# rampasek/GraphGPS

Measured on NVIDIA H100. Metric: graphs/sec GPSLayer fwd+bwd, higher is better.
Workload: dtype f32

## Files before the change

graphgps_b200/csrc/attention.cu:

```cuda
#include "kernels.cuh"

namespace gps {

namespace {

constexpr int kWarpsPerBlock = 4;

__device__ __forceinline__ int find_graph(const int* __restrict__ gptr, int B, int node) {
  int lo = 0, hi = B;
  while (hi - lo > 1) {
    int mid = (lo + hi) >> 1;
    if (gptr[mid] <= node) lo = mid; else hi = mid;
  }
  return lo;
}

template <int LPR>
__device__ __forceinline__ float group_sum(float v) {
#pragma unroll
  for (int o = LPR / 2; o > 0; o >>= 1) v += __shfl_xor_sync(0xffffffffu, v, o);
  return v;
}

__device__ __forceinline__ int warp_max_i(int v) {
#pragma unroll
  for (int o = 16; o > 0; o >>= 1) v = max(v, __shfl_xor_sync(0xffffffffu, v, o));
  return v;
}

struct DropQuad {
  Philox4 r;
  uint32_t thr;
  float keep_scale;
};
__device__ __forceinline__ void drop_quad_refresh(DropQuad& q, float p, uint64_t seed, uint64_t offset, int head, int i, int jl) {
  q.r = philox4x32(seed, offset + (uint64_t)(GPS_SITE_ATTN_P + head), ((uint64_t)i << 20) | (uint64_t)(jl >> 2));
}
__device__ __forceinline__ float drop_quad_scale(const DropQuad& q, int jl) {
  const int k = jl & 3;
  const uint32_t bits = k == 0 ? q.r.v[0] : k == 1 ? q.r.v[1] : k == 2 ? q.r.v[2] : q.r.v[3];
  return bits >= q.thr ? q.keep_scale : 0.f;
}
__device__ __forceinline__ void drop_quad_init(DropQuad& q, float p) {
  q.thr = (uint32_t)fminf(p * 4294967296.f, 4294967295.f);
  q.keep_scale = 1.f / (1.f - p);
}

template <int CH, int LPR>
__device__ __forceinline__ void load_slice(float4* dst, const float* row, int sub, int nch, bool ok) {
#pragma unroll
  for (int c = 0; c < CH; ++c) {
    int ch = sub + c * LPR;
    dst[c] = (ok && ch < nch) ? ld4(row + ch * 4) : f4zero();
  }
}
template <int CH, int LPR>
__device__ __forceinline__ void store_slice(const float4* src, float* row, int sub, int nch) {
#pragma unroll
  for (int c = 0; c < CH; ++c) {
    int ch = sub + c * LPR;
    if (ch < nch) st4(row + ch * 4, src[c]);
  }
}
template <int CH, int LPR>
__device__ __forceinline__ void store_slice_planes(const float4* src, const Planes& p, int64_t r, int64_t col0, int sub, int nch) {
  if (!p.hi) return;
#pragma unroll
  for (int c = 0; c < CH; ++c) {
    int ch = sub + c * LPR;
    if (ch < nch) planes_store4(p, r, col0 + ch * 4, src[c]);
  }
}
template <int CH>
__device__ __forceinline__ float dot_slice(const float4* a, const float4* b) {
  float s = 0.f;
#pragma unroll
  for (int c = 0; c < CH; ++c) s += a[c].x * b[c].x + a[c].y * b[c].y + a[c].z * b[c].z + a[c].w * b[c].w;
  return s;
}

struct AttnArgs {
  const int* gptr; int B; int N; int H; int hd;
  const float* Q; const float* K; const float* V; int64_t ld;
  float* O; const float* Oc; const float* dO; int64_t ldo;
  float* lse; const float* lsec; float* delta; const float* deltac;
  float* dQ; float* dK; float* dV; int64_t ldg;
  float scale; float p_drop; uint64_t seed, offset;
  const unsigned long long* offset_dev;
  Planes Op, dQp, dKp, dVp;
  int smem_rows;
};
__device__ __forceinline__ uint64_t eff_offset(const AttnArgs& a) {
  return a.offset + ((a.p_drop > 0.f && a.offset_dev) ? *a.offset_dev : 0ull);
}

struct StagedRows {
  const float* x; int64_t ldx;
  const float* y; int64_t ldy;
};
template <int RPB>
__device__ __forceinline__ StagedRows stage_rows(const AttnArgs& a, const float* X, int64_t ldX, const float* Y, int64_t ldY,
                                                 int h, float* sm) {
  const int64_t hoff = (int64_t)h * a.hd;
  StagedRows r{X + hoff, ldX, Y + hoff, ldY};
  const int r0 = blockIdx.x * RPB;
  if (a.smem_rows <= 0 || r0 >= a.N) return r;
  const int last = min(r0 + RPB, a.N) - 1;
  const int kmin = a.gptr[find_graph(a.gptr, a.B, r0)];
  const int R = a.gptr[find_graph(a.gptr, a.B, last) + 1] - kmin;
  if (R > a.smem_rows) return r;
  const int pitch = a.hd + 4, nch = a.hd >> 2;
  float* sx = sm;
  float* sy = sm + (int64_t)a.smem_rows * pitch;
  for (int idx = threadIdx.x; idx < R * nch; idx += blockDim.x) {
    const int row = idx / nch, c = idx - row * nch;
    st4(sx + row * pitch + c * 4, ld4(X + (int64_t)(kmin + row) * ldX + hoff + c * 4));
    st4(sy + row * pitch + c * 4, ld4(Y + (int64_t)(kmin + row) * ldY + hoff + c * 4));
  }
  __syncthreads();
  r.x = sx - (int64_t)kmin * pitch; r.ldx = pitch;
  r.y = sy - (int64_t)kmin * pitch; r.ldy = pitch;
  return r;
}

template <int CH, int LPR>
__global__ void __launch_bounds__(kWarpsPerBlock * 32) k_attn_fwd(AttnArgs a) {
  extern __shared__ float attn_sm[];
  constexpr int RPW = 32 / LPR;
  const int warp = threadIdx.x >> 5, lane = threadIdx.x & 31;
  const int sub = lane % LPR, rloc = lane / LPR;
  const int h = blockIdx.y;
  const int i = (blockIdx.x * kWarpsPerBlock + warp) * RPW + rloc;
  const bool row_ok = i < a.N;
  const int nch = a.hd / 4;
  const uint64_t offs = eff_offset(a);
  int gs = 0, n = 0;
  if (row_ok) {
    int g = find_graph(a.gptr, a.B, i);
    gs = a.gptr[g];
    n = a.gptr[g + 1] - gs;
  }
  const int nloop = warp_max_i(n);
  const int64_t hoff = (int64_t)h * a.hd;
  float4 q[CH], o[CH];
  load_slice<CH, LPR>(q, a.Q + (int64_t)(row_ok ? i : 0) * a.ld + hoff, sub, nch, row_ok);
#pragma unroll
  for (int c = 0; c < CH; ++c) {
    q[c] = f4scale(q[c], a.scale);
    o[c] = f4zero();
  }
  float m = -INFINITY, l = 0.f;
  const bool use_drop = a.p_drop > 0.f;
  DropQuad dq;
  drop_quad_init(dq, a.p_drop);
  const StagedRows kv = stage_rows<RPW * kWarpsPerBlock>(a, a.K, a.ld, a.V, a.ld, h, attn_sm);
  float4 kc[CH], vc[CH];
  load_slice<CH, LPR>(kc, kv.x + (int64_t)gs * kv.ldx, sub, nch, n > 0);
  load_slice<CH, LPR>(vc, kv.y + (int64_t)gs * kv.ldy, sub, nch, n > 0);
  for (int jl = 0; jl < nloop; ++jl) {
    if (use_drop && (jl & 3) == 0) drop_quad_refresh(dq, a.p_drop, a.seed, offs, h, i, jl);
    const bool valid = jl < n;
    const bool nvalid = jl + 1 < n;
    const int jn = gs + (nvalid ? jl + 1 : 0);
    float4 kn[CH], vn[CH];
    load_slice<CH, LPR>(kn, kv.x + (int64_t)jn * kv.ldx, sub, nch, nvalid);
    load_slice<CH, LPR>(vn, kv.y + (int64_t)jn * kv.ldy, sub, nch, nvalid);
    float s = group_sum<LPR>(dot_slice<CH>(q, kc));
    s = valid ? s : -INFINITY;
    const float m_new = fmaxf(m, s);
    const float corr = (m_new == -INFINITY) ? 1.f : __expf(m - m_new);
    const float p = valid ? __expf(s - m_new) : 0.f;
    l = l * corr + p;
    const float pd = use_drop ? p * drop_quad_scale(dq, jl) : p;
#pragma unroll
    for (int c = 0; c < CH; ++c) {
      o[c].x = o[c].x * corr + pd * vc[c].x;
      o[c].y = o[c].y * corr + pd * vc[c].y;
      o[c].z = o[c].z * corr + pd * vc[c].z;
      o[c].w = o[c].w * corr + pd * vc[c].w;
      kc[c] = kn[c];
      vc[c] = vn[c];
    }
    m = m_new;
  }
  if (row_ok) {
    const float inv = 1.f / l;
#pragma unroll
    for (int c = 0; c < CH; ++c) o[c] = f4scale(o[c], inv);
    store_slice<CH, LPR>(o, a.O + (int64_t)i * a.ldo + hoff, sub, nch);
    store_slice_planes<CH, LPR>(o, a.Op, i, hoff, sub, nch);
    if (sub == 0) a.lse[(int64_t)i * a.H + h] = m + __logf(l);
  }
}

__global__ void k_attn_delta(AttnArgs a) {
  const int64_t t = ((int64_t)blockIdx.x * blockDim.x + threadIdx.x) >> 3;
  const int sub = threadIdx.x & 7;
  const bool ok = t < (int64_t)a.N * a.H;
  const int64_t i = ok ? t / a.H : 0;
  const int h = ok ? (int)(t - i * a.H) : 0;
  const float4* go = reinterpret_cast<const float4*>(a.dO + i * a.ldo + (int64_t)h * a.hd);
  const float4* oo = reinterpret_cast<const float4*>(a.Oc + i * a.ldo + (int64_t)h * a.hd);
  float acc = 0.f;
  if (ok)
    for (int c = sub; c < a.hd / 4; c += 8) {
      const float4 x = __ldg(go + c), y = __ldg(oo + c);
      acc += x.x * y.x + x.y * y.y + x.z * y.z + x.w * y.w;
    }
  acc += __shfl_xor_sync(0xffffffffu, acc, 4);
  acc += __shfl_xor_sync(0xffffffffu, acc, 2);
  acc += __shfl_xor_sync(0xffffffffu, acc, 1);
  if (ok && sub == 0) a.delta[t] = acc;
}

template <int CH, int LPR>
__device__ __forceinline__ void attn_bwd_q_body(const AttnArgs& a, float* attn_sm) {
  constexpr int RPW = 32 / LPR;
  const int warp = threadIdx.x >> 5, lane = threadIdx.x & 31;
  const int sub = lane % LPR, rloc = lane / LPR;
  const int h = blockIdx.y;
  const int i = (blockIdx.x * kWarpsPerBlock + warp) * RPW + rloc;
  const bool row_ok = i < a.N;
  const int nch = a.hd / 4;
  const uint64_t offs = eff_offset(a);
  int gs = 0, n = 0;
  if (row_ok) {
    int g = find_graph(a.gptr, a.B, i);
    gs = a.gptr[g];
    n = a.gptr[g + 1] - gs;
  }
  const int nloop = warp_max_i(n);
  const int64_t hoff = (int64_t)h * a.hd;
  const int ir = row_ok ? i : 0;
  float4 q[CH], go[CH], gq[CH];
  load_slice<CH, LPR>(q, a.Q + (int64_t)ir * a.ld + hoff, sub, nch, row_ok);
  load_slice<CH, LPR>(go, a.dO + (int64_t)ir * a.ldo + hoff, sub, nch, row_ok);
  {
    const float dl = row_ok ? a.deltac[(int64_t)i * a.H + h] : 0.f;
#pragma unroll
    for (int c = 0; c < CH; ++c) gq[c] = f4zero();
    const float lse = row_ok ? a.lsec[(int64_t)i * a.H + h] : 0.f;
#pragma unroll
    for (int c = 0; c < CH; ++c) q[c] = f4scale(q[c], a.scale);
    const bool use_drop = a.p_drop > 0.f;
    DropQuad dq;
    drop_quad_init(dq, a.p_drop);
    const StagedRows kv = stage_rows<RPW * kWarpsPerBlock>(a, a.K, a.ld, a.V, a.ld, h, attn_sm);
    float4 kk[CH], vv[CH];
    load_slice<CH, LPR>(kk, kv.x + (int64_t)gs * kv.ldx, sub, nch, n > 0);
    load_slice<CH, LPR>(vv, kv.y + (int64_t)gs * kv.ldy, sub, nch, n > 0);
    for (int jl = 0; jl < nloop; ++jl) {
      if (use_drop && (jl & 3) == 0) drop_quad_refresh(dq, a.p_drop, a.seed, offs, h, i, jl);
      const bool valid = jl < n;
      const bool nvalid = jl + 1 < n;
      const int jn = gs + (nvalid ? jl + 1 : 0);
      float4 kn[CH], vn[CH];
      load_slice<CH, LPR>(kn, kv.x + (int64_t)jn * kv.ldx, sub, nch, nvalid);
      load_slice<CH, LPR>(vn, kv.y + (int64_t)jn * kv.ldy, sub, nch, nvalid);
      float s = dot_slice<CH>(q, kk), dp = dot_slice<CH>(go, vv);
#pragma unroll
      for (int ofs = LPR / 2; ofs > 0; ofs >>= 1) {
        s += __shfl_xor_sync(0xffffffffu, s, ofs);
        dp += __shfl_xor_sync(0xffffffffu, dp, ofs);
      }
      const float p = valid ? __expf(s - lse) : 0.f;
      const float ds = p * (dp * (use_drop ? drop_quad_scale(dq, jl) : 1.f) - dl);
#pragma unroll
      for (int c = 0; c < CH; ++c) {
        gq[c].x += ds * kk[c].x;
        gq[c].y += ds * kk[c].y;
        gq[c].z += ds * kk[c].z;
        gq[c].w += ds * kk[c].w;
        kk[c] = kn[c];
        vv[c] = vn[c];
      }
    }
  }
  if (row_ok) {
#pragma unroll
    for (int c = 0; c < CH; ++c) gq[c] = f4scale(gq[c], a.scale);
    store_slice<CH, LPR>(gq, a.dQ + (int64_t)i * a.ldg + hoff, sub, nch);
    store_slice_planes<CH, LPR>(gq, a.dQp, i, hoff, sub, nch);
  }
}

template <int CH, int LPR>
__device__ __forceinline__ void attn_bwd_kv_body(const AttnArgs& a, float* attn_sm) {
  constexpr int RPW = 32 / LPR;
  const int warp = threadIdx.x >> 5, lane = threadIdx.x & 31;
  const int sub = lane % LPR, rloc = lane / LPR;
  const int h = blockIdx.y;
  const int j = (blockIdx.x * kWarpsPerBlock + warp) * RPW + rloc;
  const bool row_ok = j < a.N;
  const int nch = a.hd / 4;
  const uint64_t offs = eff_offset(a);
  int gs = 0, n = 0;
  if (row_ok) {
    int g = find_graph(a.gptr, a.B, j);
    gs = a.gptr[g];
    n = a.gptr[g + 1] - gs;
  }
  const int nloop = warp_max_i(n);
  const int jl = j - gs;
  const int64_t hoff = (int64_t)h * a.hd;
  const int jr = row_ok ? j : 0;
  float4 kk[CH], vv[CH], gk[CH], gv[CH];
  load_slice<CH, LPR>(kk, a.K + (int64_t)jr * a.ld + hoff, sub, nch, row_ok);
  load_slice<CH, LPR>(vv, a.V + (int64_t)jr * a.ld + hoff, sub, nch, row_ok);
#pragma unroll
  for (int c = 0; c < CH; ++c) {
    gk[c] = f4zero();
    gv[c] = f4zero();
  }
  const StagedRows qd = stage_rows<RPW * kWarpsPerBlock>(a, a.Q, a.ld, a.dO, a.ldo, h, attn_sm);
  float4 q[CH], go[CH];
  load_slice<CH, LPR>(q, qd.x + (int64_t)gs * qd.ldx, sub, nch, n > 0);
  load_slice<CH, LPR>(go, qd.y + (int64_t)gs * qd.ldy, sub, nch, n > 0);
  for (int il = 0; il < nloop; ++il) {
    const bool valid = il < n;
    const int i = gs + (valid ? il : 0);
    const bool nvalid = il + 1 < n;
    const int in_ = gs + (nvalid ? il + 1 : 0);
    float4 qn[CH], gon[CH];
    load_slice<CH, LPR>(qn, qd.x + (int64_t)in_ * qd.ldx, sub, nch, nvalid);
    load_slice<CH, LPR>(gon, qd.y + (int64_t)in_ * qd.ldy, sub, nch, nvalid);
    float s = dot_slice<CH>(q, kk), dp = dot_slice<CH>(go, vv);
#pragma unroll
    for (int ofs = LPR / 2; ofs > 0; ofs >>= 1) {
      s += __shfl_xor_sync(0xffffffffu, s, ofs);
      dp += __shfl_xor_sync(0xffffffffu, dp, ofs);
    }
    const float lse = valid ? a.lsec[(int64_t)i * a.H + h] : 0.f;
    const float dl = valid ? a.deltac[(int64_t)i * a.H + h] : 0.f;
    const float p = valid ? __expf(s * a.scale - lse) : 0.f;
    float dsc = 1.f;
    if (a.p_drop > 0.f) {
      DropQuad dq;
      drop_quad_init(dq, a.p_drop);
      drop_quad_refresh(dq, a.p_drop, a.seed, offs, h, i, jl);
      dsc = drop_quad_scale(dq, jl);
    }
    const float pd = p * dsc;
    const float ds = p * (dp * dsc - dl) * a.scale;
#pragma unroll
    for (int c = 0; c < CH; ++c) {
      gk[c].x += ds * q[c].x; gk[c].y += ds * q[c].y; gk[c].z += ds * q[c].z; gk[c].w += ds * q[c].w;
      gv[c].x += pd * go[c].x; gv[c].y += pd * go[c].y; gv[c].z += pd * go[c].z; gv[c].w += pd * go[c].w;
      q[c] = qn[c];
      go[c] = gon[c];
    }
  }
  if (row_ok) {
    store_slice<CH, LPR>(gk, a.dK + (int64_t)j * a.ldg + hoff, sub, nch);
    store_slice<CH, LPR>(gv, a.dV + (int64_t)j * a.ldg + hoff, sub, nch);
    store_slice_planes<CH, LPR>(gk, a.dKp, j, hoff, sub, nch);
    store_slice_planes<CH, LPR>(gv, a.dVp, j, hoff, sub, nch);
  }
}

template <int CH, int LPR>
__global__ void __launch_bounds__(kWarpsPerBlock * 32) k_attn_bwd(AttnArgs a) {
  extern __shared__ float attn_sm[];
  if (blockIdx.z == 0) attn_bwd_kv_body<CH, LPR>(a, attn_sm);
  else attn_bwd_q_body<CH, LPR>(a, attn_sm);
}

enum { KFWD = 0, KBWD = 1 };

constexpr int kStageBytes = 72 * 1024;

template <int CH, int LPR>
static void launch_one(int which, const AttnArgs& a0, cudaStream_t stream) {
  constexpr int RPW = 32 / LPR;
  AttnArgs a = a0;
  static const bool stage_on = [] {
    const char* e = getenv("GPS_B200_ATTN_STAGE");
    return e && e[0] == '1';
  }();
  const int pitch = a.hd + 4;
  a.smem_rows = (stage_on && a.B > 0 && a.N < 64LL * a.B) ? kStageBytes / (2 * pitch * 4) : 0;
  const size_t smem = a.smem_rows > 0 ? (size_t)2 * a.smem_rows * pitch * 4 : 0;
  static bool attr_done[2] = {false, false};
  if (smem > 0 && !attr_done[which]) {
    if (which == KFWD) cudaFuncSetAttribute(k_attn_fwd<CH, LPR>, cudaFuncAttributeMaxDynamicSharedMemorySize, kStageBytes);
    else cudaFuncSetAttribute(k_attn_bwd<CH, LPR>, cudaFuncAttributeMaxDynamicSharedMemorySize, kStageBytes);
    attr_done[which] = true;
  }
  dim3 grid((unsigned)ceil_div(a.N, (int64_t)RPW * kWarpsPerBlock), (unsigned)a.H, which == KFWD ? 1 : 2);
  dim3 block(kWarpsPerBlock * 32);
  if (which == KFWD) k_attn_fwd<CH, LPR><<<grid, block, smem, stream>>>(a);
  else k_attn_bwd<CH, LPR><<<grid, block, smem, stream>>>(a);
}

static int dispatch(int which, const AttnArgs& a, cudaStream_t stream) {
  GPS_REQUIRE(a.hd > 0 && a.hd % 4 == 0, GPS_ERR_UNSUPPORTED, "attention: head dim %d must be a multiple of 4", a.hd);
  GPS_REQUIRE(a.ld % 4 == 0 && a.ldo % 4 == 0 && (which == KFWD || a.ldg % 4 == 0), GPS_ERR_UNSUPPORTED,
              "attention: leading dimensions must be multiples of 4");
  const int nch = a.hd / 4;
  GPS_REQUIRE(nch <= 48, GPS_ERR_UNSUPPORTED, "attention: head dim %d > 192 not supported", a.hd);
  if (a.N == 0) return GPS_OK;
  int lpr = 1;
  while ((nch + lpr - 1) / lpr > 6) lpr *= 2;
  const int ch = (nch + lpr - 1) / lpr;
#define GPS_ATTN_CASE(CHV, LPRV)                                  \
  if (ch == CHV && lpr == LPRV) {                                 \
    launch_one<CHV, LPRV>(which, a, stream);                      \
    GPS_LAUNCH_CHECK();                                           \
    return GPS_OK;                                                \
  }
  GPS_ATTN_CASE(1, 1) GPS_ATTN_CASE(2, 1) GPS_ATTN_CASE(3, 1) GPS_ATTN_CASE(4, 1) GPS_ATTN_CASE(5, 1)
  GPS_ATTN_CASE(6, 1) GPS_ATTN_CASE(4, 2) GPS_ATTN_CASE(5, 2) GPS_ATTN_CASE(6, 2) GPS_ATTN_CASE(4, 4)
  GPS_ATTN_CASE(5, 4) GPS_ATTN_CASE(6, 4) GPS_ATTN_CASE(4, 8) GPS_ATTN_CASE(5, 8) GPS_ATTN_CASE(6, 8)
#undef GPS_ATTN_CASE
  set_error("attention: no kernel for head dim %d", a.hd);
  return GPS_ERR_UNSUPPORTED;
}

}

int attention_fwd(const GpsGraph& g, int64_t heads, int64_t hd, const float* Q, const float* K, const float* V,
                  int64_t ld, float* O, int64_t ldo, float* lse, float p_drop, uint64_t seed, uint64_t offset,
                  cudaStream_t stream, const unsigned long long* offset_dev, Planes Op) {
  AttnArgs a{};
  a.offset_dev = offset_dev;
  a.Op = Op;
  a.gptr = g.graph_ptr; a.B = (int)g.B; a.N = (int)g.N; a.H = (int)heads; a.hd = (int)hd;
  a.Q = Q; a.K = K; a.V = V; a.ld = ld; a.O = O; a.ldo = ldo; a.lse = lse;
  a.scale = 1.f / sqrtf((float)hd); a.p_drop = p_drop; a.seed = seed; a.offset = offset;
  return dispatch(KFWD, a, stream);
}

int attention_bwd(const GpsGraph& g, int64_t heads, int64_t hd, const float* Q, const float* K, const float* V,
                  int64_t ld, const float* O, const float* dO, int64_t ldo, const float* lse, float* delta,
                  float* dQ, float* dK, float* dV, int64_t ldg, float p_drop, uint64_t seed, uint64_t offset,
                  cudaStream_t stream, const unsigned long long* offset_dev, Planes dQp, Planes dKp, Planes dVp) {
  AttnArgs a{};
  a.offset_dev = offset_dev;
  a.dQp = dQp; a.dKp = dKp; a.dVp = dVp;
  a.gptr = g.graph_ptr; a.B = (int)g.B; a.N = (int)g.N; a.H = (int)heads; a.hd = (int)hd;
  a.Q = Q; a.K = K; a.V = V; a.ld = ld; a.Oc = O; a.dO = dO; a.ldo = ldo; a.lsec = lse;
  a.delta = delta; a.deltac = delta; a.dQ = dQ; a.dK = dK; a.dV = dV; a.ldg = ldg;
  a.scale = 1.f / sqrtf((float)hd); a.p_drop = p_drop; a.seed = seed; a.offset = offset;
  if (a.N == 0) return GPS_OK;
  const int64_t nt = (int64_t)a.N * a.H * 8;
  k_attn_delta<<<(unsigned)ceil_div(nt, (int64_t)256), 256, 0, stream>>>(a);
  GPS_LAUNCH_CHECK();
  return dispatch(KBWD, a, stream);
}

}
```

graphgps_b200/csrc/kernels.cuh:

```cuda
#pragma once
#include "common.cuh"

namespace gps {

struct BnView {
  const float* mean = nullptr;
  const float* invstd = nullptr;
  const float* gamma = nullptr;
  const float* beta = nullptr;
  int mode = 0;
  const double* sums = nullptr;
  double inv_n = 0.0, unbias = 1.0;
  int64_t d = 0;
  float* save_mean = nullptr;
  float* save_invstd = nullptr;
  float* running_mean = nullptr;
  float* running_var = nullptr;
  long long* nbt = nullptr;
};

struct DropCfg {
  float p = 0.f;
  uint64_t seed = 0, offset = 0;
  int site = 0;
  const unsigned long long* offset_dev = nullptr;
};

int bn_act_residual(const float* z, int64_t ldz, const float* R, float* out, int64_t rows, int64_t d,
                    BnView bn, int act, DropCfg drop, double* stats, cudaStream_t stream, Planes outp = Planes());
int bn_act_residual2(const float* zx, const float* Rx, float* outx, int64_t N, BnView bnx, DropCfg dropx, double* statsx,
                     const float* ze, const float* Re, float* oute, int64_t E, BnView bne, DropCfg drope, Planes outep,
                     int64_t d, int act, cudaStream_t stream);
int bn_combine(const float* a, BnView bna, const float* b, BnView bnb, float* out, int64_t rows, int64_t d,
               cudaStream_t stream, Planes outp = Planes());

int bn_bwd_reduce(const float* g, int64_t ldg, const float* z, int64_t ldz, int64_t rows, int64_t d, BnView bn,
                  int act , DropCfg drop, double* sums, cudaStream_t stream);
int bn_bwd_apply(const float* g, int64_t ldg, const float* z, int64_t ldz, int64_t rows, int64_t d, BnView bn,
                 int act, DropCfg drop, const double* sums, float* out, int64_t ldo, float* grad_gamma,
                 float* grad_beta, cudaStream_t stream, bool accumulate = false, Planes outp = Planes());
int bn_bwd_apply_chain(const float* g, int64_t ldg, const float* z, int64_t ldz, int64_t rows, int64_t d, BnView bn,
                       const double* sums, float* out, int64_t ldo, float* grad_gamma, float* grad_beta, bool accumulate,
                       Planes outp, const float* z2, int64_t ldz2, BnView bn2, int act2, DropCfg drop2, double* sums2,
                       cudaStream_t stream);
int add3(const float* a, int64_t lda, const float* b, int64_t ldb, const float* c, int64_t ldc, float* out,
         int64_t ldo, int64_t rows, int64_t d, cudaStream_t stream);
int colsum(const float* a, int64_t lda, int64_t rows, int64_t d, float* out, cudaStream_t stream);
int copy2d(const float* src, int64_t lds, float* dst, int64_t ldd, int64_t rows, int64_t d, cudaStream_t stream);

int gatedgcn_fwd(const GpsGraph& g, int64_t d, const float* Ax, const float* Bx, const float* Dx,
                 const float* Ex, int64_t ldy, float* Ce, float* xt, double* stats_x, double* stats_e,
                 cudaStream_t stream, const float* rho = nullptr);
int gatedgcn_bwd_dst(const GpsGraph& g, int64_t d, const float* g_xt, int64_t ldg, const float* ehat,
                     const float* Bx, int64_t ldy, float* g_e, float* g_num, float* g_Dx,
                     cudaStream_t stream, Planes g_e_p = Planes(), Planes g_Dx_p = Planes(), const float* rho = nullptr,
                     float* g_den = nullptr);
int gatedgcn_bwd_src(const GpsGraph& g, int64_t d, const float* g_e, const float* ehat, const float* g_num,
                     float* g_Ex, float* g_Bx, int64_t ldg, cudaStream_t stream, Planes g_Ex_p = Planes(),
                     Planes g_Bx_p = Planes(), const float* rho = nullptr);

int64_t eslap_wgrad_chunk(int64_t E);
int eslap_fwd(const GpsGraph& g, const float* pe, int64_t k, int64_t d, int act, const float* w1, const float* b1,
              const float* w2, const float* b2, float* r, float* rho, cudaStream_t stream);
int eslap_bwd(const GpsGraph& g, const float* pe, int64_t k, int64_t d, int act, const float* g_num, const float* g_den,
              const float* Bx, int64_t ldy, const float* ehat, const float* r, const float* rho, const float* w1,
              const float* b1, const float* w2, float* gz, float* gr, float* part, float* grad_pe, float* gw1,
              float* gb1, float* gw2, float* gb2, bool accumulate, cudaStream_t stream);
int gine_fwd(const GpsGraph& g, int64_t d, const float* x, const float* e, float eps, float* out,
             cudaStream_t stream, Planes outp = Planes());
int gine_bwd_dst(const GpsGraph& g, int64_t d, const float* x, const float* e, const float* g_o, float* g_e,
                 cudaStream_t stream);
int gine_bwd_src(const GpsGraph& g, int64_t d, const float* g_e, const float* g_o, float eps, const float* add,
                 float* g_x, cudaStream_t stream);

int gcn_dinv(const GpsGraph& g, float* dinv, cudaStream_t stream);
int gcn_fwd(const GpsGraph& g, int64_t d, const float* Y, int64_t ldy, const float* dinv, const float* bias,
            const float* x, float* xloc, DropCfg drop, double* stats, cudaStream_t stream);
int gcn_bwd(const GpsGraph& g, int64_t d, const float* g_h, const float* dinv, float* gY, int64_t ldg,
            cudaStream_t stream, Planes gYp = Planes());

int attention_fwd(const GpsGraph& g, int64_t heads, int64_t hd, const float* Q, const float* K, const float* V,
                  int64_t ld, float* O, int64_t ldo, float* lse, float p_drop, uint64_t seed, uint64_t offset,
                  cudaStream_t stream, const unsigned long long* offset_dev = nullptr, Planes Op = Planes());
int attention_bwd(const GpsGraph& g, int64_t heads, int64_t hd, const float* Q, const float* K, const float* V,
                  int64_t ld, const float* O, const float* dO, int64_t ldo, const float* lse, float* delta,
                  float* dQ, float* dK, float* dV, int64_t ldg, float p_drop, uint64_t seed, uint64_t offset,
                  cudaStream_t stream, const unsigned long long* offset_dev = nullptr, Planes dQp = Planes(),
                  Planes dKp = Planes(), Planes dVp = Planes());

void attention_tc_set_debug(float* buf);
bool attention_tc_supported(int64_t hd);
int64_t attention_tc_hd_pad(int64_t hd);
int attention_tc_fwd(const GpsGraph& g, int64_t heads, int64_t hd, Planes qkv, float* O, int64_t ldo, Planes Op, float* lse,
                     float p_drop, uint64_t seed, uint64_t offset, const unsigned long long* offset_dev, int precision,
                     cudaStream_t stream);

}
```

graphgps_b200/csrc/layer.cu:

```cuda
#include <stdarg.h>
#include <string.h>

#include <algorithm>
#include <atomic>

#include "gemm.cuh"
#include "kernels.cuh"

namespace gps {

int perf_supported(int64_t dim_head, int64_t features);
int64_t perf_mp();
int perf_prep(const float* P, int64_t m, float* Pn, const GpsGraph& g, int64_t H, int* nmax, float* gmax, int* argk,
              cudaStream_t st);
int perf_features_fwd(float* fq, float* fk, const float* Q, const float* K, const GpsGraph& g, int64_t H, int64_t m,
                      float* gmax, int* argq, int* argk, cudaStream_t st);
int perf_linattn_fwd(const GpsGraph& g, int64_t H, int64_t m, const int* nmax, const float* qf, const float* kf,
                     const float* V, const float* gmax, float* O, cudaStream_t st);
int perf_linattn_bwd(const GpsGraph& g, int64_t H, int64_t m, const int* nmax, const float* qf, const float* kf,
                     const float* V, const float* gmax, const float* gO, float* g_qf, float* g_kf, float* gV,
                     float* ggmax, cudaStream_t st);
int perf_features_bwd(float* g_fq, float* g_fk, const float* fq, const float* fk, const float* Q, const float* K,
                      float* gQ, float* gK, const GpsGraph& g, int64_t H, int64_t m, const int* argq, const int* argk,
                      float* ggmax, cudaStream_t st);
// ... 284 lines not shown
  GPS_REQUIRE(a->act == GPS_ACT_RELU || a->act == GPS_ACT_GELU, GPS_ERR_ARG, "unknown activation %d", a->act);
  GPS_REQUIRE(a->dropout >= 0.f && a->dropout < 1.f && a->attn_dropout >= 0.f && a->attn_dropout < 1.f,
              GPS_ERR_ARG, "dropout probabilities must be in [0,1)");
  P->train = a->training != 0;
  P->prec = a->precision;
  P->dropout.p = P->train && a->dropout > 0.f ? a->dropout : 0.f;
  P->dropout.seed = a->seed;
  P->dropout.offset = a->offset;
  P->dropout.offset_dev = (const unsigned long long*)a->offset_dev;
  P->pa = P->train ? a->attn_dropout : 0.f;
  P->grads_accumulate = (a->reserved0 & 2) != 0;
  P->grads_prezeroed = (a->reserved0 & 1) != 0 || P->grads_accumulate;
  list_weights(a, P);
  const int64_t N = P->N, E = P->E, d = P->d;
  const bool gelu = a->act == GPS_ACT_GELU;

  Arena S(bind ? a->saved : nullptr, a->saved_bytes);
  P->bnbuf = S.alloc<float>(P->nbn * 2 * d);
  if (P->Wy) {
    P->Wcat = S.alloc<float>(P->Wy * d);
    P->bcat = S.alloc<float>(P->Wy);
    P->Y1 = S.alloc<float>(N * P->Wy);
  }
  if (P->gated) {
    P->ehat = S.alloc<float>(E * d);
    P->xt = S.alloc<float>(N * d);
    if (P->eslap) {
      P->pe_r = S.alloc<float>(E);
      P->pe_rho = S.alloc<float>(E);
    }
  }
  if (P->gine) {
    P->agg = S.alloc<float>(N * d);
    P->h1 = S.alloc<float>(N * d);
    if (gelu) P->h1_pre = S.alloc<float>(N * d);
  }
  if (P->gcn) P->dinv = S.alloc<float>(N);
  const bool loc = P->gated || P->gine || P->gcn;
  if (loc && !P->nonorm) P->xloc = S.alloc<float>(N * d);
  if (P->attn) {
    P->O = S.alloc<float>(N * d);
    P->lse = S.alloc<float>(N * P->H);
    if (!P->nonorm) P->hA = S.alloc<float>(N * d);
  }
  if (P->perf) {
    const int64_t NH = N * P->H, BH = a->graph.B * P->H;
    P->pQ = S.alloc<float>(N * P->inner);
    P->pK = S.alloc<float>(N * P->inner);
    P->pV = S.alloc<float>(N * P->inner);
    P->pfq = S.alloc<float>(NH * P->mp);
    P->pfk = S.alloc<float>(NH * P->mp);
    P->pPn = S.alloc<float>(P->mp * a->perf_dim_head);
    P->pgmax = S.alloc<float>(BH);
    P->pargq = S.alloc<int>(NH);
    P->pargk = S.alloc<int>(BH);
    P->pnmax = S.alloc<int>(1);
    P->pden = S.alloc<float>(NH);
    P->perf_pairwise = a->graph.B > 0 && N <= 48 * a->graph.B;
    P->O = S.alloc<float>(N * P->inner);
    if (!P->nonorm) P->hA = S.alloc<float>(N * d);
  }
  P->s = S.alloc<float>(N * d);
  P->hid = S.alloc<float>(N * 2 * d);
  if (gelu) P->hid_pre = S.alloc<float>(N * 2 * d);
  if (!P->nonorm) P->t = S.alloc<float>(N * d);
  P->use_planes = (d % 8 == 0) && (!P->perf || P->inner % 8 == 0);
  const bool lo = a->precision == GPS_PREC_FP32;
  auto mkplanes = [&](Arena& A, int64_t rows, int64_t cols) {
    Planes q;
    q.ld = round_up(cols, 8);
    q.hi = A.alloc<__nv_bfloat16>(rows * q.ld + 8);
    q.lo = lo ? A.alloc<__nv_bfloat16>(rows * q.ld + 8) : nullptr;
    return q;
  };
  if (P->use_planes) {
    const int64_t kout = P->perf ? P->inner : d;
    P->x_p = caller_planes(a->x_planes_in, d, a->precision);
    if (!P->x_p.hi) P->x_p = mkplanes(S, N, d);
    if (P->gated || P->gine) {
      P->e_p = caller_planes(a->e_planes_in, d, a->precision);
      if (!P->e_p.hi) P->e_p = mkplanes(S, E, d);
    }
    if (P->attn || P->perf) P->O_p = mkplanes(S, N, kout);
    P->attn_tc = P->attn && attention_tc_supported(P->hd) && a->graph.B > 0 && N >= 64 * a->graph.B;
    if (P->attn_tc) P->qkv_p = mkplanes(S, N, 3 * P->H * attention_tc_hd_pad(P->hd));
    P->s_p = mkplanes(S, N, d);
    P->hid_p = mkplanes(S, N, 2 * d);
    if (P->gine) {
      P->agg_p = mkplanes(S, N, d);
      P->h1_p = mkplanes(S, N, d);
    }
    Arena Wa(bind ? a->wplanes : nullptr, a->wplanes_bytes);
    Arena& WA = bind && a->wplanes != nullptr ? Wa : S;
    const int64_t w0 = WA.used;
    for (int i = 0; i < P->nweights; ++i) {
      const LayerWeight& w = P->weights[i];
      if (w.row0 == 0) P->*w.planes = mkplanes(WA, w.planes == &Plan::Wcat_p ? P->Wy : w.lin.rows, w.cols);
    }
    P->wplanes_bytes = WA.used - w0;
    GPS_REQUIRE(!Wa.overflow, GPS_ERR_ARG, "wplanes buffer too small (%lld < %lld)", (long long)a->wplanes_bytes,
                (long long)P->wplanes_bytes);
  }
  P->saved_bytes = S.used;
  GPS_REQUIRE(!S.overflow, GPS_ERR_ARG, "saved buffer too small (%lld < %lld)", (long long)a->saved_bytes,
              (long long)S.used);

  Arena F(bind ? a->workspace : nullptr, a->workspace_bytes);
  P->fstats = F.alloc<double>(P->nbn * 2 * d);
  if (P->nonorm && loc) {
    P->xloc = (P->attn || P->perf) ? F.alloc<float>(N * d) : P->s;
  }
  P->fwd_bytes = F.used;

  Arena Bk(bind ? a->workspace : nullptr, a->workspace_bytes);
  P->bsums = Bk.alloc<double>(P->nbn * 2 * d);
  if (!P->nonorm) P->g_t = Bk.alloc<float>(N * d);
  P->g_hid = Bk.alloc<float>(N * 2 * d);
  P->g_s = Bk.alloc<float>(N * d);
  P->g_tmp = Bk.alloc<float>(N * d);
  if (a->dropout > 0.f || (P->perf && a->attn_dropout > 0.f)) {
    P->g_tmp2 = Bk.alloc<float>(N * d);
    P->g_tmp3 = Bk.alloc<float>(N * d);
  }
  if (loc && !P->nonorm) P->g_xloc = Bk.alloc<float>(N * d);
  if (P->attn) {
    if (!P->nonorm) P->g_hA = Bk.alloc<float>(N * d);
    P->g_O = Bk.alloc<float>(N * d);
    P->delta = Bk.alloc<float>(N * P->H);
  }
  if (P->perf) {
    const int64_t NH = N * P->H, BH = a->graph.B * P->H;
    if (!P->nonorm) P->g_hA = Bk.alloc<float>(N * d);
    P->g_O = Bk.alloc<float>(N * P->inner);
    P->g_pfq = Bk.alloc<float>(NH * P->mp);
    P->g_pfk = Bk.alloc<float>(NH * P->mp);
    P->g_pQ = Bk.alloc<float>(N * P->inner);
    P->g_pK = Bk.alloc<float>(N * P->inner);
    P->g_pV = Bk.alloc<float>(N * P->inner);
    P->g_pgmax = Bk.alloc<float>(BH);
    P->g_pden = Bk.alloc<float>(NH);
    P->g_xp = Bk.alloc<float>(N * d);
  }
  if (P->Wy) {
    P->gY1 = Bk.alloc<float>(N * P->Wy);
    P->gWcat = Bk.alloc<float>(P->Wy * d + P->Wy);
    P->gbcat = P->gWcat ? P->gWcat + P->Wy * d : nullptr;
  }
  if (P->gated) {
    P->g_e = Bk.alloc<float>(E * d);
    P->g_num = Bk.alloc<float>(N * d);
    if (P->eslap) {
      P->g_den = Bk.alloc<float>(N * d);
      P->pe_gz = Bk.alloc<float>(E);
      P->pe_gr = Bk.alloc<float>(E);
      P->pe_part = Bk.alloc<float>(ceil_div(E, eslap_wgrad_chunk(E)) * (3 * d + 1));
    }
  }
  if (P->gine) {
    P->g_h1 = Bk.alloc<float>(N * d);
    P->g_agg = Bk.alloc<float>(N * d);
    P->g_xl = Bk.alloc<float>(N * d);
  }
  if (P->use_planes) {
    P->gt_p = mkplanes(Bk, N, d);
    P->ghid_p = mkplanes(Bk, N, 2 * d);
    if ((P->attn || P->perf) && !P->nonorm) P->ghA_p = mkplanes(Bk, N, d);
    if (P->nonorm) P->gs_p = mkplanes(Bk, N, d);
// ... 886 lines not shown
```

Measured before the change: 339,200.

## Add per-graph shared-memory tiled attention backward for small graphs

Removes the env-gated smem row staging and adds a new backward kernel for batches of small graphs. Each CTA stages the Q, dO, K and V tiles of its graph in shared memory, builds the probability and dS matrices once, then computes dQ, dK and dV from shared memory. For whole graphs it derives delta inside the kernel, which skips the separate delta kernel. This is meant to cut repeated global K/V/Q reloads and the doubled kv/q passes. It may lose occupancy from 48KB of smem per block and adds more complex chunked tiling for larger graphs.

After: 348,400, median of 6. 2.7% higher.

```diff
diff --git a/graphgps_b200/csrc/attention.cu b/graphgps_b200/csrc/attention.cu
--- a/graphgps_b200/csrc/attention.cu
+++ b/graphgps_b200/csrc/attention.cu
@@ -88,44 +88,14 @@
   float scale; float p_drop; uint64_t seed, offset;
   const unsigned long long* offset_dev;
   Planes Op, dQp, dKp, dVp;
-  int smem_rows;
 };
 __device__ __forceinline__ uint64_t eff_offset(const AttnArgs& a) {
   return a.offset + ((a.p_drop > 0.f && a.offset_dev) ? *a.offset_dev : 0ull);
 }
 
-struct StagedRows {
-  const float* x; int64_t ldx;
-  const float* y; int64_t ldy;
-};
-template <int RPB>
-__device__ __forceinline__ StagedRows stage_rows(const AttnArgs& a, const float* X, int64_t ldX, const float* Y, int64_t ldY,
-                                                 int h, float* sm) {
-  const int64_t hoff = (int64_t)h * a.hd;
-  StagedRows r{X + hoff, ldX, Y + hoff, ldY};
-  const int r0 = blockIdx.x * RPB;
-  if (a.smem_rows <= 0 || r0 >= a.N) return r;
-  const int last = min(r0 + RPB, a.N) - 1;
-  const int kmin = a.gptr[find_graph(a.gptr, a.B, r0)];
-  const int R = a.gptr[find_graph(a.gptr, a.B, last) + 1] - kmin;
-  if (R > a.smem_rows) return r;
-  const int pitch = a.hd + 4, nch = a.hd >> 2;
-  float* sx = sm;
-  float* sy = sm + (int64_t)a.smem_rows * pitch;
-  for (int idx = threadIdx.x; idx < R * nch; idx += blockDim.x) {
-    const int row = idx / nch, c = idx - row * nch;
-    st4(sx + row * pitch + c * 4, ld4(X + (int64_t)(kmin + row) * ldX + hoff + c * 4));
-    st4(sy + row * pitch + c * 4, ld4(Y + (int64_t)(kmin + row) * ldY + hoff + c * 4));
-  }
-  __syncthreads();
-  r.x = sx - (int64_t)kmin * pitch; r.ldx = pitch;
-  r.y = sy - (int64_t)kmin * pitch; r.ldy = pitch;
-  return r;
-}
 
 template <int CH, int LPR>
 __global__ void __launch_bounds__(kWarpsPerBlock * 32) k_attn_fwd(AttnArgs a) {
-  extern __shared__ float attn_sm[];
   constexpr int RPW = 32 / LPR;
   const int warp = threadIdx.x >> 5, lane = threadIdx.x & 31;
   const int sub = lane % LPR, rloc = lane / LPR;
@@ -153,18 +123,19 @@
   const bool use_drop = a.p_drop > 0.f;
   DropQuad dq;
   drop_quad_init(dq, a.p_drop);
-  const StagedRows kv = stage_rows<RPW * kWarpsPerBlock>(a, a.K, a.ld, a.V, a.ld, h, attn_sm);
+  const float* kx = a.K + hoff;
+  const float* vx = a.V + hoff;
   float4 kc[CH], vc[CH];
-  load_slice<CH, LPR>(kc, kv.x + (int64_t)gs * kv.ldx, sub, nch, n > 0);
-  load_slice<CH, LPR>(vc, kv.y + (int64_t)gs * kv.ldy, sub, nch, n > 0);
+  load_slice<CH, LPR>(kc, kx + (int64_t)gs * a.ld, sub, nch, n > 0);
+  load_slice<CH, LPR>(vc, vx + (int64_t)gs * a.ld, sub, nch, n > 0);
   for (int jl = 0; jl < nloop; ++jl) {
     if (use_drop && (jl & 3) == 0) drop_quad_refresh(dq, a.p_drop, a.seed, offs, h, i, jl);
     const bool valid = jl < n;
     const bool nvalid = jl + 1 < n;
     const int jn = gs + (nvalid ? jl + 1 : 0);
     float4 kn[CH], vn[CH];
-    load_slice<CH, LPR>(kn, kv.x + (int64_t)jn * kv.ldx, sub, nch, nvalid);
-    load_slice<CH, LPR>(vn, kv.y + (int64_t)jn * kv.ldy, sub, nch, nvalid);
+    load_slice<CH, LPR>(kn, kx + (int64_t)jn * a.ld, sub, nch, nvalid);
+    load_slice<CH, LPR>(vn, vx + (int64_t)jn * a.ld, sub, nch, nvalid);
     float s = group_sum<LPR>(dot_slice<CH>(q, kc));
     s = valid ? s : -INFINITY;
     const float m_new = fmaxf(m, s);
@@ -214,7 +185,7 @@
 }
 
 template <int CH, int LPR>
-__device__ __forceinline__ void attn_bwd_q_body(const AttnArgs& a, float* attn_sm) {
+__device__ __forceinline__ void attn_bwd_q_body(const AttnArgs& a) {
   constexpr int RPW = 32 / LPR;
   const int warp = threadIdx.x >> 5, lane = threadIdx.x & 31;
   const int sub = lane % LPR, rloc = lane / LPR;
@@ -245,18 +216,19 @@
     const bool use_drop = a.p_drop > 0.f;
     DropQuad dq;
     drop_quad_init(dq, a.p_drop);
-    const StagedRows kv = stage_rows<RPW * kWarpsPerBlock>(a, a.K, a.ld, a.V, a.ld, h, attn_sm);
+    const float* kx = a.K + hoff;
+    const float* vx = a.V + hoff;
     float4 kk[CH], vv[CH];
-    load_slice<CH, LPR>(kk, kv.x + (int64_t)gs * kv.ldx, sub, nch, n > 0);
-    load_slice<CH, LPR>(vv, kv.y + (int64_t)gs * kv.ldy, sub, nch, n > 0);
+    load_slice<CH, LPR>(kk, kx + (int64_t)gs * a.ld, sub, nch, n > 0);
+    load_slice<CH, LPR>(vv, vx + (int64_t)gs * a.ld, sub, nch, n > 0);
     for (int jl = 0; jl < nloop; ++jl) {
       if (use_drop && (jl & 3) == 0) drop_quad_refresh(dq, a.p_drop, a.seed, offs, h, i, jl);
       const bool valid = jl < n;
       const bool nvalid = jl + 1 < n;
       const int jn = gs + (nvalid ? jl + 1 : 0);
       float4 kn[CH], vn[CH];
-      load_slice<CH, LPR>(kn, kv.x + (int64_t)jn * kv.ldx, sub, nch, nvalid);
-      load_slice<CH, LPR>(vn, kv.y + (int64_t)jn * kv.ldy, sub, nch, nvalid);
+      load_slice<CH, LPR>(kn, kx + (int64_t)jn * a.ld, sub, nch, nvalid);
+      load_slice<CH, LPR>(vn, vx + (int64_t)jn * a.ld, sub, nch, nvalid);
       float s = dot_slice<CH>(q, kk), dp = dot_slice<CH>(go, vv);
 #pragma unroll
       for (int ofs = LPR / 2; ofs > 0; ofs >>= 1) {
@@ -285,7 +257,7 @@
 }
 
 template <int CH, int LPR>
-__device__ __forceinline__ void attn_bwd_kv_body(const AttnArgs& a, float* attn_sm) {
+__device__ __forceinline__ void attn_bwd_kv_body(const AttnArgs& a) {
   constexpr int RPW = 32 / LPR;
   const int warp = threadIdx.x >> 5, lane = threadIdx.x & 31;
   const int sub = lane % LPR, rloc = lane / LPR;
@@ -312,18 +284,19 @@
     gk[c] = f4zero();
     gv[c] = f4zero();
   }
-  const StagedRows qd = stage_rows<RPW * kWarpsPerBlock>(a, a.Q, a.ld, a.dO, a.ldo, h, attn_sm);
+  const float* qx = a.Q + hoff;
+  const float* ox = a.dO + hoff;
   float4 q[CH], go[CH];
-  load_slice<CH, LPR>(q, qd.x + (int64_t)gs * qd.ldx, sub, nch, n > 0);
-  load_slice<CH, LPR>(go, qd.y + (int64_t)gs * qd.ldy, sub, nch, n > 0);
+  load_slice<CH, LPR>(q, qx + (int64_t)gs * a.ld, sub, nch, n > 0);
+  load_slice<CH, LPR>(go, ox + (int64_t)gs * a.ldo, sub, nch, n > 0);
   for (int il = 0; il < nloop; ++il) {
     const bool valid = il < n;
     const int i = gs + (valid ? il : 0);
     const bool nvalid = il + 1 < n;
     const int in_ = gs + (nvalid ? il + 1 : 0);
     float4 qn[CH], gon[CH];
-    load_slice<CH, LPR>(qn, qd.x + (int64_t)in_ * qd.ldx, sub, nch, nvalid);
-    load_slice<CH, LPR>(gon, qd.y + (int64_t)in_ * qd.ldy, sub, nch, nvalid);
+    load_slice<CH, LPR>(qn, qx + (int64_t)in_ * a.ld, sub, nch, nvalid);
+    load_slice<CH, LPR>(gon, ox + (int64_t)in_ * a.ldo, sub, nch, nvalid);
     float s = dot_slice<CH>(q, kk), dp = dot_slice<CH>(go, vv);
 #pragma unroll
     for (int ofs = LPR / 2; ofs > 0; ofs >>= 1) {
@@ -360,45 +333,216 @@
 
 template <int CH, int LPR>
 __global__ void __launch_bounds__(kWarpsPerBlock * 32) k_attn_bwd(AttnArgs a) {
-  extern __shared__ float attn_sm[];
-  if (blockIdx.z == 0) attn_bwd_kv_body<CH, LPR>(a, attn_sm);
-  else attn_bwd_q_body<CH, LPR>(a, attn_sm);
+  if (blockIdx.z == 0) attn_bwd_kv_body<CH, LPR>(a);
+  else attn_bwd_q_body<CH, LPR>(a);
+}
+
+constexpr int kGraphThreads = 128;
+constexpr int kGraphSmemBytes = 48 * 1024;
+constexpr int kGraphMaxRows = 64;
+
+__host__ __device__ constexpr int tile_pitch(int hd) { return ((hd / 4) & 1) ? hd : hd + 4; }
+__host__ __device__ constexpr int graph_tile_rows(int hd) {
+  int s = kGraphMaxRows;
+  while (s > 4 && (4 * s * tile_pitch(hd) + 2 * s * s) * 4 > kGraphSmemBytes) s -= 4;
+  return s;
+}
+static_assert(graph_tile_rows(76) >= 32, "a C3 tile must hold 32 rows");
+__host__ __device__ constexpr int graph_bwd_smem_floats(int hd) {
+  return 4 * graph_tile_rows(hd) * tile_pitch(hd) + 2 * graph_tile_rows(hd) * graph_tile_rows(hd);
+}
+
+__device__ __forceinline__ void stage_tile(float* dst, int pitch, const float* X, int64_t ldx, int row0, int rows, int nch) {
+  for (int idx = threadIdx.x; idx < rows * nch; idx += kGraphThreads) {
+    const int r = idx / nch, c = idx - r * nch;
+    st4(dst + r * pitch + c * 4, ld4(X + (int64_t)(row0 + r) * ldx + c * 4));
+  }
+}
+__device__ __forceinline__ float dot4(float4 a, float4 b) { return a.x * b.x + a.y * b.y + a.z * b.z + a.w * b.w; }
+__device__ __forceinline__ float warp_max_f(float v) {
+#pragma unroll
+  for (int o = 16; o > 0; o >>= 1) v = fmaxf(v, __shfl_xor_sync(0xffffffffu, v, o));
+  return v;
+}
+__device__ __forceinline__ float drop_scale_at(DropQuad& dq, const AttnArgs& a, uint64_t offs, int h, int i, int jl) {
+  drop_quad_refresh(dq, a.p_drop, a.seed, offs, h, i, jl);
+  return drop_quad_scale(dq, jl);
+}
+
+__device__ __forceinline__ bool owned_rows(int gs, int ge, int S, int& own0, int& own1) {
+  const int r0 = blockIdx.x * 32;
+  if (ge == gs) return false;
+  if (ge - gs <= S) {
+    own0 = gs; own1 = ge;
+    return gs >= r0;
+  }
+  own0 = max(gs, r0); own1 = min(ge, r0 + 32);
+  return true;
+}
+__device__ __forceinline__ int first_graph(const AttnArgs& a) { return find_graph(a.gptr, a.B, blockIdx.x * 32); }
+__device__ __forceinline__ bool graph_in_cta(const AttnArgs& a, int g) {
+  return g < a.B && a.gptr[g] < min(blockIdx.x * 32 + 32, a.N);
+}
+
+enum { kWhole = 0, kDq = 1, kDkv = 2 };
+__device__ __forceinline__ void graph_bwd_tile(const AttnArgs& a, float* sm, DropQuad& dq, int h, uint64_t offs, int gs, int qa,
+                                               int nq, int ka, int nk, int mode, bool first, bool last) {
+  const int hd = a.hd, nch = hd / 4, pitch = tile_pitch(hd), S = graph_tile_rows(hd);
+  const int64_t hoff = (int64_t)h * hd;
+  float* sQ = sm;
+  float* sG = sQ + S * pitch;
+  float* sK = sG + S * pitch;
+  float* sV = sK + S * pitch;
+  float* sP = sV + S * pitch;
+  float* sD = sP + S * S;
+  stage_tile(sQ, pitch, a.Q + hoff, a.ld, qa, nq, nch);
+  stage_tile(sG, pitch, a.dO + hoff, a.ldo, qa, nq, nch);
+  stage_tile(sK, pitch, a.K + hoff, a.ld, ka, nk, nch);
+  stage_tile(sV, pitch, a.V + hoff, a.ld, ka, nk, nch);
+  __syncthreads();
+  const int warp = threadIdx.x >> 5, lane = threadIdx.x & 31;
+  const bool use_drop = a.p_drop > 0.f;
+  for (int r = warp; r < nq; r += kGraphThreads / 32) {
+    const int i = qa + r;
+    const float lse = a.lsec[(int64_t)i * a.H + h];
+    const float4* q = reinterpret_cast<const float4*>(sQ + r * pitch);
+    const float4* go = reinterpret_cast<const float4*>(sG + r * pitch);
+    float p[2], dp[2], ms[2];
+    float dsum = 0.f;
+#pragma unroll
+    for (int t = 0; t < 2; ++t) {
+      const int j = lane + 32 * t;
+      p[t] = 0.f; dp[t] = 0.f; ms[t] = 1.f;
+      if (j < nk) {
+        const float4* k = reinterpret_cast<const float4*>(sK + j * pitch);
+        const float4* v = reinterpret_cast<const float4*>(sV + j * pitch);
+        float4 s = f4zero(), d = f4zero();
+#pragma unroll 4
+        for (int c = 0; c < nch; ++c) {
+          s = f4fma(q[c], k[c], s);
+          d = f4fma(go[c], v[c], d);
+        }
+        p[t] = __expf((s.x + s.y + s.z + s.w) * a.scale - lse);
+        dp[t] = d.x + d.y + d.z + d.w;
+        const float dpt = dp[t];
+        if (use_drop) ms[t] = drop_scale_at(dq, a, offs, h, i, ka - gs + j);
+        dsum += p[t] * ms[t] * dpt;
+      }
+    }
+    if (mode != kWhole) {
+      dsum = 0.f;
+      const float4* o = reinterpret_cast<const float4*>(a.Oc + (int64_t)i * a.ldo + hoff);
+      for (int c = lane; c < nch; c += 32) dsum += dot4(go[c], o[c]);
+    }
+    const float delta = warp_sum(dsum);
+#pragma unroll
+    for (int t = 0; t < 2; ++t) {
+      const int j = lane + 32 * t;
+      if (j < nk) {
+        sP[r * S + j] = p[t] * ms[t];
+        sD[r * S + j] = p[t] * (dp[t] * ms[t] - delta);
+      }
+    }
+  }
+  __syncthreads();
+  const int rows = mode == kDkv ? nk : nq;
+  for (int idx = threadIdx.x; idx < rows * nch; idx += kGraphThreads) {
+    const int r = idx / nch, c = idx - r * nch;
+    if (mode != kDkv) {
+      float4 gq = f4zero();
+      for (int j = 0; j < nk; ++j) {
+        const float ds = sD[r * S + j];
+        const float4 k = ld4(sK + j * pitch + c * 4);
+        gq.x += ds * k.x; gq.y += ds * k.y; gq.z += ds * k.z; gq.w += ds * k.w;
+      }
+      gq = f4scale(gq, a.scale);
+      float* row = a.dQ + (int64_t)(qa + r) * a.ldg + hoff + c * 4;
+      if (!first) gq = f4add(ld4(row), gq);
+      st4(row, gq);
+      if (last && a.dQp.hi) planes_store4(a.dQp, qa + r, hoff + c * 4, gq);
+    }
+    if (mode != kDq) {
+      float4 gk = f4zero(), gv = f4zero();
+      for (int i = 0; i < nq; ++i) {
+        const float ds = sD[i * S + r], pt = sP[i * S + r];
+        const float4 q = ld4(sQ + i * pitch + c * 4), go = ld4(sG + i * pitch + c * 4);
+        gk.x += ds * q.x; gk.y += ds * q.y; gk.z += ds * q.z; gk.w += ds * q.w;
+        gv.x += pt * go.x; gv.y += pt * go.y; gv.z += pt * go.z; gv.w += pt * go.w;
+      }
+      gk = f4scale(gk, a.scale);
+      float* krow = a.dK + (int64_t)(ka + r) * a.ldg + hoff + c * 4;
+      float* vrow = a.dV + (int64_t)(ka + r) * a.ldg + hoff + c * 4;
+      if (!first) {
+        gk = f4add(ld4(krow), gk);
+        gv = f4add(ld4(vrow), gv);
+      }
+      st4(krow, gk);
+      st4(vrow, gv);
+      if (last && a.dKp.hi) planes_store4(a.dKp, ka + r, hoff + c * 4, gk);
+      if (last && a.dVp.hi) planes_store4(a.dVp, ka + r, hoff + c * 4, gv);
+    }
+  }
+  __syncthreads();
+}
+
+__global__ void __launch_bounds__(kGraphThreads) k_attn_graph_bwd(AttnArgs a) {
+  extern __shared__ float4 graph_sm4[];
+  float* sm = reinterpret_cast<float*>(graph_sm4);
+  const int h = blockIdx.y, S = graph_tile_rows(a.hd);
+  const uint64_t offs = eff_offset(a);
+  DropQuad dq;
+  drop_quad_init(dq, a.p_drop);
+  for (int g = first_graph(a); graph_in_cta(a, g); ++g) {
+    const int gs = a.gptr[g], ge = a.gptr[g + 1];
+    int own0, own1;
+    if (!owned_rows(gs, ge, S, own0, own1)) continue;
+    const bool whole = ge - gs <= S;
+    const int nchunk = whole ? 1 : (ge - gs + S - 1) / S;
+    const int ntile = whole ? 1 : (own1 - own0 + S - 1) / S * 2 * nchunk;
+    for (int t = 0; t < ntile; ++t) {
+      const int oa = own0 + t / (2 * nchunk) * S, no = min(S, own1 - oa);
+      const int c = t % (2 * nchunk) % nchunk;
+      const int ca = gs + c * S, nc = min(S, ge - ca);
+      const int mode = whole ? kWhole : t % (2 * nchunk) < nchunk ? kDq : kDkv;
+      const bool kv = mode == kDkv;
+      graph_bwd_tile(a, sm, dq, h, offs, gs, kv ? ca : oa, kv ? nc : no, kv ? oa : ca, kv ? no : nc, mode, c == 0,
+                     c == nchunk - 1);
+    }
+  }
 }
 
 enum { KFWD = 0, KBWD = 1 };
 
-constexpr int kStageBytes = 72 * 1024;
-
-template <int CH, int LPR>
-static void launch_one(int which, const AttnArgs& a0, cudaStream_t stream) {
+template <int CH, int LPR>
+static void launch_one(int which, const AttnArgs& a, cudaStream_t stream) {
   constexpr int RPW = 32 / LPR;
-  AttnArgs a = a0;
-  static const bool stage_on = [] {
-    const char* e = getenv("GPS_B200_ATTN_STAGE");
-    return e && e[0] == '1';
-  }();
-  const int pitch = a.hd + 4;
-  a.smem_rows = (stage_on && a.B > 0 && a.N < 64LL * a.B) ? kStageBytes / (2 * pitch * 4) : 0;
-  const size_t smem = a.smem_rows > 0 ? (size_t)2 * a.smem_rows * pitch * 4 : 0;
-  static bool attr_done[2] = {false, false};
-  if (smem > 0 && !attr_done[which]) {
-    if (which == KFWD) cudaFuncSetAttribute(k_attn_fwd<CH, LPR>, cudaFuncAttributeMaxDynamicSharedMemorySize, kStageBytes);
-    else cudaFuncSetAttribute(k_attn_bwd<CH, LPR>, cudaFuncAttributeMaxDynamicSharedMemorySize, kStageBytes);
-    attr_done[which] = true;
-  }
   dim3 grid((unsigned)ceil_div(a.N, (int64_t)RPW * kWarpsPerBlock), (unsigned)a.H, which == KFWD ? 1 : 2);
   dim3 block(kWarpsPerBlock * 32);
-  if (which == KFWD) k_attn_fwd<CH, LPR><<<grid, block, smem, stream>>>(a);
-  else k_attn_bwd<CH, LPR><<<grid, block, smem, stream>>>(a);
-}
-
-static int dispatch(int which, const AttnArgs& a, cudaStream_t stream) {
+  if (which == KFWD) k_attn_fwd<CH, LPR><<<grid, block, 0, stream>>>(a);
+  else k_attn_bwd<CH, LPR><<<grid, block, 0, stream>>>(a);
+}
+
+static int launch_graph_bwd(const AttnArgs& a, cudaStream_t stream) {
+  const size_t smem = (size_t)graph_bwd_smem_floats(a.hd) * 4;
+  dim3 grid((unsigned)ceil_div(a.N, (int64_t)32), (unsigned)a.H);
+  k_attn_graph_bwd<<<grid, kGraphThreads, smem, stream>>>(a);
+  GPS_LAUNCH_CHECK();
+  return GPS_OK;
+}
+
+static int dispatch(int which, const GpsGraph& g, const AttnArgs& a, cudaStream_t stream) {
   GPS_REQUIRE(a.hd > 0 && a.hd % 4 == 0, GPS_ERR_UNSUPPORTED, "attention: head dim %d must be a multiple of 4", a.hd);
   GPS_REQUIRE(a.ld % 4 == 0 && a.ldo % 4 == 0 && (which == KFWD || a.ldg % 4 == 0), GPS_ERR_UNSUPPORTED,
               "attention: leading dimensions must be multiples of 4");
   const int nch = a.hd / 4;
   GPS_REQUIRE(nch <= 48, GPS_ERR_UNSUPPORTED, "attention: head dim %d > 192 not supported", a.hd);
   if (a.N == 0) return GPS_OK;
+  if (which == KBWD && attention_small_graphs(g) && nch > 6) return launch_graph_bwd(a, stream);
+  if (which == KBWD) {
+    const int64_t nt = (int64_t)a.N * a.H * 8;
+    k_attn_delta<<<(unsigned)ceil_div(nt, (int64_t)256), 256, 0, stream>>>(a);
+    GPS_LAUNCH_CHECK();
+  }
   int lpr = 1;
   while ((nch + lpr - 1) / lpr > 6) lpr *= 2;
   const int ch = (nch + lpr - 1) / lpr;
@@ -427,7 +571,7 @@
   a.gptr = g.graph_ptr; a.B = (int)g.B; a.N = (int)g.N; a.H = (int)heads; a.hd = (int)hd;
   a.Q = Q; a.K = K; a.V = V; a.ld = ld; a.O = O; a.ldo = ldo; a.lse = lse;
   a.scale = 1.f / sqrtf((float)hd); a.p_drop = p_drop; a.seed = seed; a.offset = offset;
-  return dispatch(KFWD, a, stream);
+  return dispatch(KFWD, g, a, stream);
 }
 
 int attention_bwd(const GpsGraph& g, int64_t heads, int64_t hd, const float* Q, const float* K, const float* V,
@@ -441,11 +585,7 @@
   a.Q = Q; a.K = K; a.V = V; a.ld = ld; a.Oc = O; a.dO = dO; a.ldo = ldo; a.lsec = lse;
   a.delta = delta; a.deltac = delta; a.dQ = dQ; a.dK = dK; a.dV = dV; a.ldg = ldg;
   a.scale = 1.f / sqrtf((float)hd); a.p_drop = p_drop; a.seed = seed; a.offset = offset;
-  if (a.N == 0) return GPS_OK;
-  const int64_t nt = (int64_t)a.N * a.H * 8;
-  k_attn_delta<<<(unsigned)ceil_div(nt, (int64_t)256), 256, 0, stream>>>(a);
-  GPS_LAUNCH_CHECK();
-  return dispatch(KBWD, a, stream);
-}
-
-}
+  return dispatch(KBWD, g, a, stream);
+}
+
+}
diff --git a/graphgps_b200/csrc/kernels.cuh b/graphgps_b200/csrc/kernels.cuh
--- a/graphgps_b200/csrc/kernels.cuh
+++ b/graphgps_b200/csrc/kernels.cuh
@@ -79,6 +79,7 @@
 int gcn_bwd(const GpsGraph& g, int64_t d, const float* g_h, const float* dinv, float* gY, int64_t ldg,
             cudaStream_t stream, Planes gYp = Planes());
 
+inline bool attention_small_graphs(const GpsGraph& g) { return g.B > 0 && g.N < 64 * g.B; }
 int attention_fwd(const GpsGraph& g, int64_t heads, int64_t hd, const float* Q, const float* K, const float* V,
                   int64_t ld, float* O, int64_t ldo, float* lse, float p_drop, uint64_t seed, uint64_t offset,
                   cudaStream_t stream, const unsigned long long* offset_dev = nullptr, Planes Op = Planes());
diff --git a/graphgps_b200/csrc/layer.cu b/graphgps_b200/csrc/layer.cu
--- a/graphgps_b200/csrc/layer.cu
+++ b/graphgps_b200/csrc/layer.cu
@@ -390,7 +390,7 @@
       if (!P->e_p.hi) P->e_p = mkplanes(S, E, d);
     }
     if (P->attn || P->perf) P->O_p = mkplanes(S, N, kout);
-    P->attn_tc = P->attn && attention_tc_supported(P->hd) && a->graph.B > 0 && N >= 64 * a->graph.B;
+    P->attn_tc = P->attn && attention_tc_supported(P->hd) && a->graph.B > 0 && !attention_small_graphs(a->graph);
     if (P->attn_tc) P->qkv_p = mkplanes(S, N, 3 * P->H * attention_tc_hd_pad(P->hd));
     P->s_p = mkplanes(S, N, d);
     P->hid_p = mkplanes(S, N, 2 * d);
```
